# JNP-Solutions/Slacken

Hardware: AMD Instinct MI355X
Metric: classify_throughput_150bp_standard224scale (higher is better)
Workload: dtype u64

## Files before the change

### slacken_amd/csrc/lane.hip

```cpp
#include "engine.h"

#include <algorithm>
#include <cstddef>
#include <cstdio>
#include <cstdlib>

namespace slk {

#ifndef SLK_LANE_LW
#define SLK_LANE_LW 4
#endif
constexpr int LW = SLK_LANE_LW;
constexpr int QCAP = 128;
#ifndef SLK_SBLK
#define SLK_SBLK 5
#endif
constexpr int SBLK = SLK_SBLK;
#ifndef SLK_OMAP
#define SLK_OMAP 12
#endif
constexpr int OMAP = SLK_OMAP;
constexpr int OMAP_CNT_BITS = 10;
constexpr uint32_t OMAP_CNT_MASK = (1u << OMAP_CNT_BITS) - 1;

// ... 96 lines not shown
  for (int s = 0; s < LPB; s++) {
    uint32_t bkt = ((const uint4 *)L->stash)[s * PG + g].x;
    SLK_TUNE(if (dbg & 4) bkt &= 1023u;)
    cell[s] = SLK_PROBE_LOAD((const ulonglong2 *)(cellbase + ((uint64_t)bkt << BUCKET_SHIFT)));
  }
  constexpr uint64_t GROUP_LSB = LPB == 4 ? 0x1111111111111111ULL : 0x0101010101010101ULL;
  int requeued = 0;
#pragma unroll
  for (int s = 0; s < LPB; s++) {
    const uint2 tg = *(const uint2 *)&((const uint4 *)L->stash)[s * PG + g].z;
    const uint64_t want = ((uint64_t)tg.y << 32) | tg.x;
    const bool act = want != NO_TAG;
    const bool e0 = cell[s].x == 0, e1 = cell[s].y == 0;
    const bool m0 = act && !e0 && cell_tag(T.g, cell[s].x) == want;
    const bool m1 = act && !e1 && cell_tag(T.g, cell[s].y) == want;
    if (m0 || m1) L->found[s * PG + g] = (uint32_t)((m0 ? cell[s].x : cell[s].y) & tmask);
    const bool closed = T.g.flag != 0 && c == 0 && (cell[s].x & T.g.flag) == 0;
    const uint64_t B = __ballot(m0 || m1 || e0 || e1 || !act || closed);
    uint64_t any = B;
#pragma unroll
    for (int i = 1; i < LPB; i <<= 1) any |= any >> i;
    if ((any & GROUP_LSB) != GROUP_LSB) {
      const int qj = (qhead + s * PG + g) & (QCAP - 1);
      const uint32_t m_old = L->q_meta[qj];
      const bool again = c == 0 && ((B >> (g * LPB)) & ((1u << LPB) - 1)) == 0 && (int)((m_old >> 20) & 255) < T.max_disp;
      const uint64_t k_old = L->q_key[qj];
      const uint16_t o_old = HITS ? L->q_ord[qj] : (uint16_t)0;
      const uint64_t R = __ballot(again);
      lane_wave_sync();
      if (again) {
        const int slot = (qhead + qn + requeued + __builtin_amdgcn_mbcnt_hi((uint32_t)(R >> 32), __builtin_amdgcn_mbcnt_lo((uint32_t)R, 0))) & (QCAP - 1);
        L->q_key[slot] = k_old;
        L->q_meta[slot] = m_old + (1u << 20);
        if (HITS) L->q_ord[slot] = o_old;
      }
      requeued += __popcll(R);
    }
  }
  lane_wave_sync();
  const int32_t taxon = (int32_t)L->found[lane];
  if (!SLK_TUNE_ON(2)) fold_hit<LONG>(L, ocnt, in, meta, taxon);
  if (HITS && in) {
    const uint64_t at = L->rb[meta & 63] + ord;
    hit_taxon[at] = ext_taxon(T, taxon);
    hit_meta[at] = pack_meta((int32_t)((meta >> 7) & 0x1FFF), 1, (meta >> 6) & 1);
  }
  lane_wave_sync();
  return requeued;
}

#ifndef SLK_STREAM_NT
#define SLK_STREAM_NT 0
#endif
#ifndef SLK_APPLY_ROWS
#define SLK_APPLY_ROWS 4
#endif
template <class T> __device__ __forceinline__ T SLK_STREAM_LOAD(const T *p) {
#if SLK_STREAM_NT
  return __builtin_nontemporal_load(p);
#else
  return *p;
#endif
}
template <class T> __device__ __forceinline__ void SLK_STREAM_STORE(T *p, T v) {
#if SLK_STREAM_NT
  __builtin_nontemporal_store(v, p);
#else
  *p = v;
#endif
}

__device__ __forceinline__ uint64_t lane_readlane64(uint64_t v, int src) {
  uint32_t lo = __builtin_amdgcn_readlane((uint32_t)v, src), hi = __builtin_amdgcn_readlane((uint32_t)(v >> 32), src);
  return ((uint64_t)hi << 32) | lo;
}
__device__ __forceinline__ uint32_t shard_owner(uint64_t key, uint32_t ns) {
  const uint64_t h = fmix64(key);
  return (ns & (ns - 1)) == 0 ? (uint32_t)(h & (ns - 1)) : (uint32_t)(h % ns);
}
__device__ __forceinline__ uint64_t side_load(const ShardIO &S, uint64_t batch, int lane) {
  const uint64_t i = batch * 64 + (uint64_t)lane;
  return i < S.side_n ? (uint64_t)SLK_STREAM_LOAD(&S.side_keys[i]) : 0;
}
__device__ __forceinline__ void side_probe(LaneLds *L, const TableView &T, const ShardIO &S, int lane, uint64_t batch, uint64_t key, int dbg) {
  const uint64_t base = batch * 64;
  if (base >= S.side_n) return;
  const uint64_t i = base + (uint64_t)lane;
  const bool in = i < S.side_n;
  const uint64_t h = fmix64(key);
  uint32_t home;
  uint64_t rem_hi;
  table_slot(T.g, h, home, rem_hi);
  const uint64_t tag = in ? rem_hi : ~0ULL;
  uint4 st;
  st.x = home; st.y = 0; st.z = (uint32_t)tag; st.w = (uint32_t)(tag >> 32);
  ((uint4 *)L->stash)[lane] = st;
  L->found[lane] = 0;
  lane_wave_sync();
  const int g = lane / LPB, c = lane % LPB;
  const uint64_t tmask = (1ULL << T.g.taxon_bits) - 1;
  const char *cellbase = (const char *)T.cells + c * 16;
  ulonglong2 cell[LPB];
#pragma unroll
  for (int s = 0; s < LPB; s++) {
    uint32_t bkt = ((const uint4 *)L->stash)[s * PG + g].x;
    SLK_TUNE(if (dbg & 4) bkt &= 1023u;)
    cell[s] = SLK_PROBE_LOAD((const ulonglong2 *)(cellbase + ((uint64_t)bkt << BUCKET_SHIFT)));
  }
  uint32_t unresolved = 0;
#pragma unroll
  for (int s = 0; s < LPB; s++) {
    const uint2 tg = *(const uint2 *)&((const uint4 *)L->stash)[s * PG + g].z;
    const uint64_t want = ((uint64_t)tg.y << 32) | tg.x;
    const bool act = want != ~0ULL;
    const bool e0 = cell[s].x == 0, e1 = cell[s].y == 0;
    const bool m0 = act && !e0 && cell_tag(T.g, cell[s].x) == want;
    const bool m1 = act && !e1 && cell_tag(T.g, cell[s].y) == want;
    if (m0 || m1) L->found[s * PG + g] = (uint32_t)((m0 ? cell[s].x : cell[s].y) & tmask);
    const bool closed = T.g.flag != 0 && c == 0 && (cell[s].x & T.g.flag) == 0;
    const uint64_t B = __ballot(m0 || m1 || e0 || e1 || !act || closed);
    if (((B >> (g * LPB)) & ((1u << LPB) - 1)) == 0) unresolved |= 1u << s;
  }
  lane_wave_sync();
  int32_t taxon = (int32_t)L->found[lane];
  const uint32_t ur = (uint32_t)__shfl((int)unresolved, (lane % PG) * LPB);
  if (in && ((ur >> (lane / PG)) & 1)) {
    for (int d = 1; d <= T.max_disp; d++) {
      const ulonglong2 *b = (const ulonglong2 *)(T.cells + ((uint64_t)table_bucket(T.g, home, (uint32_t)d) * CELLS));
      const uint64_t want = rem_hi | (uint64_t)d;
      bool has_empty = false, closed = false;
      int32_t hit = 0;
#pragma unroll
      for (int q = 0; q < LPB; q++) {
        const ulonglong2 v = b[q];
        has_empty |= (v.x == 0) | (v.y == 0);
        if (q == 0) closed = T.g.flag != 0 && (v.x & T.g.flag) == 0;
        if (v.x != 0 && cell_tag(T.g, v.x) == want) hit = (int32_t)(v.x & tmask);
        if (v.y != 0 && cell_tag(T.g, v.y) == want) hit = (int32_t)(v.y & tmask);
      }
      if (hit) { taxon = hit; break; }
      if (has_empty || closed) break;
    }
  }
  if (in && !SLK_TUNE_ON(128)) SLK_STREAM_STORE(&S.side_out[i], ext_taxon(T, taxon));
  lane_wave_sync();
}

template <bool HITS>
__device__ __forceinline__ void apply_rows(LaneLds *L, const ApplyJob &J, int lane, uint64_t row0, uint32_t nrows) {
  const uint32_t ns = (uint32_t)J.n_shards;
  constexpr int U = SLK_APPLY_ROWS;
  for (uint32_t b = 0; b < nrows; b += U) {
    uint64_t at[U];
    bool in[U];
#pragma unroll
    for (int u = 0; u < U; u++) {
      in[u] = false;
      at[u] = 0;
      if (b + u < nrows) {
        uint32_t off = 0;
        for (uint32_t sh = 0; sh < ns; sh++) {
          const uint4 e = J.batch_log[(row0 + b + u) * ns + sh];
          const uint32_t cnt = e.z;
          if (cnt == 0) continue;
          if ((uint32_t)lane >= off && (uint32_t)lane < off + cnt) {
            in[u] = true;
            const uint32_t i = (uint32_t)lane - off;
            at[u] = (uint64_t)sh * J.cap + (i < e.w ? e.x + i : e.y + (i - e.w));
          }
          off += cnt;
        }
      }
    }
    uint32_t meta[U];
    int32_t taxon[U];
#pragma unroll
    for (int u = 0; u < U; u++) {
      meta[u] = in[u] ? SLK_STREAM_LOAD(&J.send_meta[at[u]]) : 0u;
      taxon[u] = in[u] ? SLK_STREAM_LOAD(&J.taxa[at[u]]) : 0;
    }
#pragma unroll
    for (int u = 0; u < U; u++) {
      if (b + u < nrows) {
        int32_t t = taxon[u];
        if (in[u]) {
          if (HITS) {
            const uint64_t hat = L->rb[meta[u] & 63] + (meta[u] >> 20);
            J.A.span_taxon[hat] = t;
            J.A.span_meta[hat] = pack_meta((int32_t)((meta[u] >> 7) & 0x1FFF), 1, (meta[u] >> 6) & 1);
          }
          if (J.to_dense != nullptr && t > 0) t = t < J.n_to_dense ? J.to_dense[t] : 0;
        }
        fold_hit<false>(L, nullptr, in[u], meta[u], t);
      }
    }
    lane_wave_sync();
  }
}

template <bool HITS>
__device__ __forceinline__ void emit_batch(LaneLds *L, const FusedArgs &A, const ShardIO &S, const ApplyJob &J, int qhead, int cnt, int lane,
                                           uint64_t row, uint64_t tile, uint32_t &ch_pos, uint32_t &ch_end, uint32_t &side_j, uint64_t &side_key, int dbg) {
  SLK_TUNE(if (dbg & 256) return;)
  const bool in = lane < cnt;
  const int qi = (qhead + lane) & (QCAP - 1);
  const uint64_t key = L->q_key[qi];
  const uint32_t meta = L->q_meta[qi] | (HITS ? (uint32_t)L->q_ord[qi] << 20 : 0u);
  const uint32_t ns = (uint32_t)S.n_shards;
  const uint32_t g = ns == 1 ? 0u : shard_owner(key, ns);
  uint32_t mycount = 0, rank = 0;
  for (uint32_t sh = 0; sh < ns; sh++) {
    const uint64_t m = __ballot(in && g == sh);
    if ((uint32_t)lane == sh) mycount = (uint32_t)__popcll(m);
    if (g == sh) rank = __builtin_amdgcn_mbcnt_hi((uint32_t)(m >> 32), __builtin_amdgcn_mbcnt_lo((uint32_t)m, 0));
  }
  const uint32_t pos = ch_pos, room = ch_end - ch_pos;
  const bool need = (uint32_t)lane < ns && mycount > room;
  unsigned long long got = 0;
  if (need) got = atomicAdd(&S.cursors[lane], (unsigned long long)S.chunk);
  if (side_j < S.side_per_tile) {
    const uint64_t batch = tile * S.side_per_tile + side_j;
    const uint64_t k_now = side_key;
    side_j++;
    if (side_j < S.side_per_tile) side_key = side_load(S, batch + 1, lane);
    side_probe(L, A.T, S, lane, batch, k_now, dbg);
  }
  uint32_t fresh = 0xFFFFFFFFu;
  if (need) {
    if (got + S.chunk <= S.cap) fresh = (uint32_t)got;
    else atomicOr(A.status, 2);
  }
  if ((uint32_t)lane < ns) {
    S.batch_log[row * ns + (uint32_t)lane] = make_uint4(pos, fresh, mycount, room);
    if (need) { ch_pos = fresh == 0xFFFFFFFFu ? 0u : fresh + (mycount - room); ch_end = fresh == 0xFFFFFFFFu ? 0u : fresh + S.chunk; }
    else ch_pos = pos + mycount;
  }
  const uint32_t gpos = (uint32_t)__shfl((int)pos, (int)g), groom = (uint32_t)__shfl((int)room, (int)g), gfresh = (uint32_t)__shfl((int)fresh, (int)g);
  if (in) {
    const bool tail = rank >= groom;
    if ((!tail || gfresh != 0xFFFFFFFFu) && !SLK_TUNE_ON(32)) {
      const uint64_t at = (uint64_t)g * S.cap + (tail ? gfresh + (rank - groom) : gpos + rank);
      SLK_STREAM_STORE(&S.send_keys[at], (int64_t)key);
      SLK_STREAM_STORE(&S.send_meta[at], meta);
    }
  }
  lane_wave_sync();
}

__device__ __forceinline__ uint4 lane_node(const uint4 *nodes, int32_t ntax, int32_t t) {
  return ((uint32_t)t < (uint32_t)ntax) ? nodes[t] : make_uint4(0u, 0x40000000u + (uint32_t)t, 0x40000000u + (uint32_t)t, 0u);
}
__device__ __forceinline__ int lane_code(uint32_t c) {
  const uint32_t VM = (1u << 1) | (1u << 3) | (1u << 7) | (1u << 20) | (1u << 21);
  bool ok = ((c & 0xC0) == 0x40) && ((VM >> (c & 31)) & 1);
  uint32_t t = (c >> 1) & 3;
  t ^= t >> 1;
  return ok ? (int)t : 5;
}

__device__ __forceinline__ uint4 stream_refill(LaneLds *L, int lane, const uint8_t *seq, uint32_t p, uint32_t n, uint32_t room) {
  uint4 v[SBLK];
#pragma unroll
  for (int i = 0; i < SBLK; i++) {
    v[i] = make_uint4(0, 0, 0, 0);
    if (p + 16u * i < n) v[i] = load_block16(seq + p + 16u * i, room - (p + 16u * i));
  }
#pragma unroll
  for (int i = 1; i < SBLK; i++) L->sbuf[(i - 1) * 64 + lane] = v[i];
  return v[0];
}

#ifndef SLK_PACKED_STREAM
#define SLK_PACKED_STREAM 1
#endif
#ifndef SLK_PACK_ROUNDS
#define SLK_PACK_ROUNDS 2
#endif
constexpr uint32_t PACK_MAX_SPAN = 10880;
constexpr uint32_t PACK_WORDS = PACK_MAX_SPAN / 16 + 1;
constexpr int PACK_LOADS = (PACK_MAX_SPAN + 1023) / 1024;
static_assert((size_t)PACK_WORDS * 6 <= (size_t)(SBLK - 1) * 64 * 16, "the packed tile lives in the lane-wise stream's LDS slots");
__device__ __forceinline__ void pack16(const uint4 v, uint32_t &codes, uint32_t &valid) {
  const uint32_t VM = (1u << 1) | (1u << 3) | (1u << 7) | (1u << 20) | (1u << 21);
  const uint32_t w[4] = {v.x, v.y, v.z, v.w};
  codes = 0; valid = 0;
#pragma unroll
  for (int d = 0; d < 4; d++) {
    uint32_t t = (w[d] >> 1) & 0x03030303u;
    t ^= (t >> 1) & 0x01010101u;
    t = (t | (t >> 6) | (t >> 12) | (t >> 18)) & 0xFFu;
    codes |= t << (8 * d);
#pragma unroll
    for (int b = 0; b < 4; b++) {
      const uint32_t c = (w[d] >> (8 * b)) & 0xFFu;
      const uint32_t ok = (((c & 0xC0u) == 0x40u) ? 1u : 0u) & (VM >> (c & 31u));
      valid |= (ok & 1u) << (4 * d + b);
    }
  }
}
__device__ __forceinline__ uint2 packed_take(const uint32_t *pcodes, const uint16_t *pvalid, uint32_t s) {
  const uint32_t wi = s >> 4, bo = s & 15u;
  const uint64_t c64 = (uint64_t)pcodes[wi] | ((uint64_t)pcodes[wi + 1] << 32);
  const uint32_t v32 = (uint32_t)pvalid[wi] | ((uint32_t)pvalid[wi + 1] << 16);
  return make_uint2((uint32_t)(c64 >> (2 * bo)), (v32 >> bo) & 0xFFFFu);
}

#ifndef SLK_LANE_WPS
#define SLK_LANE_WPS 0
#endif
#if SLK_LANE_WPS > 0
#define LANE_BOUNDS __launch_bounds__(LW * 64, SLK_LANE_WPS)
#else
#define LANE_BOUNDS __launch_bounds__(LW * 64) __attribute__((amdgpu_waves_per_eu(4)))
#endif

__device__ __forceinline__ int route_by_length(uint64_t len, uint32_t long_max, uint32_t b0, uint32_t b1, uint32_t b2, uint32_t seg_min_len,
                                               uint32_t wave_min, uint32_t wave_ratio_q10) {
  if (long_max != 0 && len <= long_max) return (len > b0) + (len > b1) + (len > b2);
  if (seg_min_len != 0 && len >= seg_min_len) return HandOn::SEG;
  int c = HandOn::WAVE_CLASSES - 1;
  for (uint64_t b = ((uint64_t)wave_min * wave_ratio_q10) >> 10; c > 0 && len >= b; b = (b * wave_ratio_q10) >> 10) c--;
  return HandOn::WAVE0 + c;
}
__device__ __attribute__((noinline)) void hand_on(unsigned long long *hdr, uint32_t *lists, uint64_t stride, uint64_t long_cap, uint32_t long_max,
                                                  uint32_t b0, uint32_t b1, uint32_t b2, uint32_t seg_min_len, uint32_t wave_min,
                                                  uint32_t wave_ratio_q10, const uint64_t *offsets, const uint64_t *mate_offsets, bool dfr,
                                                  bool too_long, uint64_t r, int lane, bool from_long) {
  const uint64_t DM = __ballot(dfr);
  int route = from_long ? HandOn::LATE : HandOn::REST;
  if (!from_long && dfr && too_long) {
    uint64_t len = offsets[r + 1] - offsets[r];
    if (mate_offsets) len += mate_offsets[r + 1] - mate_offsets[r];
    route = route_by_length(len, long_max, b0, b1, b2, seg_min_len, wave_min, wave_ratio_q10);
  }
  if (!from_long && lane == 0) atomicAdd(&hdr[HandOn::HANDED], (unsigned long long)__popcll(DM));
  for (int l = from_long ? HandOn::LATE : 0; l <= HandOn::LATE; l++) {
    const uint64_t M = __ballot(dfr && route == l);
    if (M == 0) continue;
    const int leader = __ffsll((long long)M) - 1;
    unsigned long long at = 0;
    if (lane == leader) at = atomicAdd(&hdr[HandOn::count_word(l)], (unsigned long long)__popcll(M));
    at = lane_readlane64(at, leader);
    if (dfr && route == l)
      lists[HandOn::list_at(l, stride, long_cap) + at + __builtin_amdgcn_mbcnt_hi((uint32_t)(M >> 32), __builtin_amdgcn_mbcnt_lo((uint32_t)M, 0))] = (uint32_t)r;
  }
}

__global__ void __launch_bounds__(256) route_kernel(FusedArgs A) {
// ... 223 lines not shown
      if (paired) n2 = (uint32_t)(A.mate_offsets[r + 1] - A.mate_offsets[r]);
    }
    bool too_long = have && ((uint64_t)n + n2 > max_len);
    bool fin = !have || too_long;
    uint64_t row = 0, row0 = 0;
    if (MODE == LANE_EMIT && tile < etiles) row = row0 = (span_region(A.offsets, A.mate_offsets, tile * 64) >> 6) + tile;
    const uint64_t rbase = (HITS && have) ? span_region(A.offsets, A.mate_offsets, r) : 0;
    if (HITS && MODE != LANE_EMIT) L->rb[lane] = rbase;
#pragma unroll
    for (int s = 0; s < OMAP; s++) L->omap[s * 64 + lane] = 0;
    if (LONG) {
#pragma unroll
      for (int s = 0; s < OMAP; s++) ocnt[s * 64 + lane] = 0;
    }
    L->o_flags[lane] = 0;
    if (MODE == LANE_EMIT && tile < atiles) {
      const uint64_t r2 = tile * 64 + lane;
      const bool have2 = r2 < Jp->A.R;
      const uint2 tr = Jp->tile_rows[tile];
      if (HITS) L->rb[lane] = have2 ? span_region(Jp->A.offsets, Jp->A.mate_offsets, r2) : 0;
      lane_wave_sync();
      apply_rows<HITS>(L, *Jp, lane, tr.x, tr.y);
      const bool dfr2 = have2 && (Jp->defer[r2] != 0 || (L->o_flags[lane] & 0x80000000u));
      const uint64_t DM = __ballot(dfr2);
      if (DM != 0 && lane == 0) atomicAdd(Jp->n_deferred, (unsigned long long)__popcll(DM));
      if (have2) {
        if (dfr2) {
          Jp->defer[r2] = 1;
          if (Jp->A.out_nh) Jp->A.out_nh[r2] = 0;
          if (HITS) Jp->A.span_count[r2] = 0;
        } else {
          const int2 ri = Jp->read_info[r2];
          resolve_lane<HITS, false>(L, nullptr, Jp->A, lane, r2, L->o_flags[lane], ri.x, ri.y, 0, dbg);
        }
      }
      lane_wave_sync();
    }
    uint32_t pos = 0;
    int mate = 0;
    uint32_t cur = 0, b1 = 0, b2 = 0, b3 = 0;
    int sb = 1;
    bool packed = false;
    uint32_t s0 = 0;
    uint32_t *const pcodes = (uint32_t *)L->sbuf;
    uint16_t *const pvalid = (uint16_t *)(pcodes + PACK_WORDS);
    constexpr bool CAN_PACK = SLK_PACKED_STREAM && !LONG && MODE == LANE_LOCAL;
    if (CAN_PACK && !paired) {
      const uint64_t t0 = tile * 64, t1 = min(A.R, t0 + 64);
      const uint64_t span_o = A.offsets[t0], span = A.offsets[t1] - span_o;
      if (span <= PACK_MAX_SPAN && __ballot(!fin) != 0) {
        packed = true;
        s0 = have ? (uint32_t)(A.offsets[r] - span_o) : 0;
        const uint8_t *tb = A.bases + span_o;
        const uint32_t troom = clamp_room(bases_end - span_o), sp = (uint32_t)span;
        constexpr int PG0 = (PACK_LOADS + SLK_PACK_ROUNDS - 1) / SLK_PACK_ROUNDS;
#pragma unroll
        for (int j0 = 0; j0 < PACK_LOADS; j0 += PG0) {
          uint4 v[PG0];
#pragma unroll
          for (int j = 0; j < PG0; j++) {
            const uint32_t cb = (uint32_t)(j0 + j) * 1024u + (uint32_t)lane * 16u;
            v[j] = make_uint4(0, 0, 0, 0);
            if (j0 + j < PACK_LOADS && cb < sp) v[j] = load_block16(tb + cb, troom - cb);
          }
#pragma unroll
          for (int j = 0; j < PG0; j++) {
            const uint32_t cb = (uint32_t)(j0 + j) * 1024u + (uint32_t)lane * 16u;
            if (j0 + j < PACK_LOADS && cb < sp + 16u) {
              uint32_t cw, vw;
              pack16(v[j], cw, vw);
              pcodes[cb >> 4] = cw;
              pvalid[cb >> 4] = (uint16_t)vw;
            }
          }
        }
        lane_wave_sync();
      }
    }
    if (!fin && n > 0) {
      if (CAN_PACK && packed) {
        const uint2 pk = packed_take(pcodes, pvalid, s0);
        cur = pk.x; b1 = pk.y;
      } else {
        uint4 v = stream_refill(L, lane, seq, 0, n, room);
        cur = v.x; b1 = v.y; b2 = v.z; b3 = v.w;
      }
    }
    int run_class = 0;
    uint32_t run_len = 0, nvalid = 0;
    uint64_t fwd = 0, rc = 0;
    uint64_t k1 = ~0ULL, p1 = ~0ULL, p2 = ~0ULL, m41 = ~0ULL;
    uint64_t pre = ~0ULL;
    uint64_t cur_val = 0;
    int32_t cur_run = 0;
    bool first = true, have_last = false;
    uint64_t last_key = 0;
    int32_t total = 0, np = 0, nhits = 0;
    uint32_t side_j = (MODE == LANE_EMIT && S.side_n != 0 && tile < etiles) ? 0u : 0xFFFFFFFFu;
    uint64_t side_key = (MODE == LANE_EMIT && S.side_n != 0 && S.side_per_tile != 0 && tile < etiles) ? side_load(S, tile * S.side_per_tile, lane) : 0;
    int qn = 0;
    int qhead = 0;
    int tphase = 0;

    const uint32_t VM = (1u << 1) | (1u << 3) | (1u << 7) | (1u << 20) | (1u << 21);
    while (__ballot(!fin) != 0) {
      if (!W5 && tphase == 0) pre = ~0ULL;
      const bool act = !fin;
      const bool is_end = pos >= n;
      bool okc;
      uint32_t t;
      if (CAN_PACK && packed) {
        t = cur & 3u;
        okc = (b1 & 1u) != 0;
      } else {
        const uint32_t c = cur & 0xFF;
        okc = ((c & 0xC0) == 0x40) && ((VM >> (c & 31)) & 1);
        t = (c >> 1) & 3;
        t ^= t >> 1;
      }
      const int cls = is_end ? -1 : (okc ? 1 : 0);
      const bool run_end = act && run_len > 0 && cls != run_class;
      const bool seqrun = run_class == 1 && nvalid >= (uint32_t)k;
      const bool seq_close = run_end && seqrun;
      const bool amb_close = run_end && !seqrun && run_len >= (uint32_t)k;
      const int32_t ord0 = nhits;
      total += amb_close ? (int32_t)run_len - (k - 1) : 0;
      if (HITS && amb_close) {
        A.span_meta[rbase + ord0] = pack_meta((int32_t)run_len - (k - 1), 2, 0);
        A.span_taxon[rbase + ord0] = -1;
      }
      nhits += amb_close ? 1 : 0;
      first = first && !amb_close;
      const uint64_t ekey = cur_val;
      const int32_t ekmers = cur_run;
      run_len = run_end ? 0u : run_len;
      const bool proc = act && !is_end;
      const bool new_run = proc && run_len == 0;
      run_class = new_run ? cls : run_class;
      nvalid = new_run ? 0u : nvalid;
      cur_run = (new_run || seq_close) ? 0 : cur_run;
      run_len += proc ? 1u : 0u;
      const bool nt = proc && okc;
      nvalid += nt ? 1u : 0u;
      fwd = (fwd << 2) | ((uint64_t)t << P.sh);
      rc = ((rc >> 2) | ((uint64_t)(3 - t) << 62)) & P.keep;
      const bool havekey = nt && nvalid >= (uint32_t)m;
      const uint64_t canon = (P.canonical && rc < fwd) ? rc : fwd;
      const uint64_t key = (canon ^ P.xmask) & P.smask;
      uint64_t minv;
      if (W5) {
        const uint64_t p = lmin64(key, k1);
        const uint64_t m4 = lmin64(p, p2);
        minv = lmin64(key, m41);
        k1 = key; p2 = p1; p1 = p; m41 = m4;
      } else {
        const uint64_t kk = havekey ? key : ~0ULL;
        pre = lmin64(pre, kk);
        minv = (tphase == w - 1) ? pre : lmin64(pre, win[(tphase + 1) * 64 + lane]);
        win[tphase * 64 + lane] = kk;
      }
      const bool havewin = havekey && nvalid >= (uint32_t)k;
      const bool start = havewin && cur_run == 0;
      const bool same = havewin && cur_run != 0 && minv == cur_val;
      const bool change = havewin && cur_run != 0 && minv != cur_val;
      const bool emit = seq_close || change;
      cur_val = (start || change) ? minv : cur_val;
      cur_run = (start || change) ? 1 : (same ? cur_run + 1 : cur_run);
      pos += proc ? 1u : 0u;
      const bool refill = proc && (pos & 15) == 0;
      if (CAN_PACK && packed) {
        cur = proc ? (cur >> 2) : cur;
        b1 = proc ? (b1 >> 1) : b1;
        if (__ballot(refill) != 0) {
          if (refill && pos < n) {
            const uint2 pk = packed_take(pcodes, pvalid, s0 + pos);
            cur = pk.x; b1 = pk.y;
          }
        }
      } else {
        const bool nextdw = proc && (pos & 3) == 0;
        cur = nextdw ? b1 : (proc ? (cur >> 8) : cur);
        b1 = nextdw ? b2 : b1;
        b2 = nextdw ? b3 : b2;
        if (__ballot(refill) != 0) {
          if (refill) {
            if (pos < n) {
              uint4 v;
              if (sb < SBLK) { v = L->sbuf[(sb - 1) * 64 + lane]; sb++; }
              else { v = stream_refill(L, lane, seq, pos, n, room); sb = 1; }
              cur = v.x; b1 = v.y; b2 = v.z; b3 = v.w;
            }
          }
        }
      }
      const bool at_end = act && is_end;
      if (__ballot(at_end) != 0) {
        if (at_end) {
          if (mate == 0 && paired) {
            if (HITS) {
              const int32_t ordb = ord0 + ((amb_close || emit) ? 1 : 0);
              A.span_meta[rbase + ordb] = pack_meta(-(k - 1), 3, 0);
              A.span_taxon[rbase + ordb] = -2;
            }
            nhits++;
            first = false;
            mate = 1;
            const uint64_t o2 = A.mate_offsets[r];
            seq = A.mate_bases + o2; n = (uint32_t)(A.mate_offsets[r + 1] - o2); room = clamp_room(mates_end - o2); pos = 0;
            if (n > 0) {
              uint4 v = stream_refill(L, lane, seq, 0, n, room);
              sb = 1;
              cur = v.x; b1 = v.y; b2 = v.z; b3 = v.w;
            }
          } else {
            fin = true;
          }
        }
      }
      if (!W5) {
        if (tphase == w - 1) {
          uint64_t sm = ~0ULL;
          for (int j = w - 1; j >= 0; j--) { sm = lmin64(sm, win[j * 64 + lane]); win[j * 64 + lane] = sm; }
          tphase = 0;
        } else {
          tphase++;
        }
      }
      const bool distinct = emit && (first || !(have_last && ekey == last_key));
      last_key = emit ? ekey : last_key;
      have_last = have_last || emit;
      first = first && !emit;
      total += emit ? ekmers : 0;
      np += emit ? 1 : 0;
      nhits += emit ? 1 : 0;
      uint64_t E = __ballot(emit);
      if (E != 0) {
        if (emit) {
          int slot = (qhead + qn + __builtin_amdgcn_mbcnt_hi((uint32_t)(E >> 32), __builtin_amdgcn_mbcnt_lo((uint32_t)E, 0))) & (QCAP - 1);
          L->q_key[slot] = ekey;
          if (HITS) L->q_ord[slot] = (uint16_t)ord0;
          L->q_meta[slot] = (uint32_t)lane | (distinct ? 64u : 0u) | ((uint32_t)ekmers << 7);
        }
        qn += __popcll(E);
        while (qn >= 64) {
          lane_wave_sync();
          int back = 0;
          if (MODE == LANE_EMIT) emit_batch<HITS>(L, A, S, *Jp, qhead, 64, lane, row++, tile, ch_pos, ch_end, side_j, side_key, dbg);
          else if (!SLK_TUNE_ON(1)) back = probe_batch<HITS, LONG>(L, ocnt, A.T, qhead, qn, 64, lane, dbg, A.span_meta, A.span_taxon);
          qhead = (qhead + 64) & (QCAP - 1);
          qn += back - 64;
        }
      }
    }
    while (qn > 0) {
      lane_wave_sync();
      const int cnt = min(qn, 64);
      int back = 0;
      if (MODE == LANE_EMIT) emit_batch<HITS>(L, A, S, *Jp, qhead, cnt, lane, row++, tile, ch_pos, ch_end, side_j, side_key, dbg);
      else if (!SLK_TUNE_ON(1)) back = probe_batch<HITS, LONG>(L, ocnt, A.T, qhead, qn, cnt, lane, dbg, A.span_meta, A.span_taxon);
      qhead = (qhead + cnt) & (QCAP - 1);
      qn += back - cnt;
    }
    lane_wave_sync();
    if (MODE == LANE_EMIT) {
      if (tile < etiles) {
        if (have) S.read_info[r] = make_int2(total, nhits);
        if (lane == 0) S.tile_rows[tile] = make_uint2((uint32_t)row0, (uint32_t)(row - row0));
      }
      while (side_j < S.side_per_tile) {
        const uint64_t batch = tile * S.side_per_tile + side_j;
        const uint64_t k_now = side_key;
        side_j++;
        if (side_j < S.side_per_tile) side_key = side_load(S, batch + 1, lane);
        side_probe(L, A.T, S, lane, batch, k_now, dbg);
      }
    }

    if (MODE == LANE_LOCAL) {
      const uint32_t oflags = have ? L->o_flags[lane] : 0u;
      const bool dfr = have && (too_long || (oflags & 0x80000000u));
      if (__ballot(dfr) != 0)
        hand_on(A.hand_hdr, A.hand_lists, A.hand_stride, A.hand_long_cap, A.long_max, A.long_bound[0], A.long_bound[1], A.long_bound[2],
                A.seg_min_len, A.wave_min, A.wave_ratio_q10, A.offsets, A.mate_offsets, dfr, too_long, r, lane, LONG);
      if (have && !dfr) resolve_lane<HITS, LONG>(L, ocnt, A, lane, r, oflags, total, nhits, np, dbg);
    } else {
      if (have && too_long) defer[r] = 1;
    }
    lane_wave_sync();
  }
  if (MODE == LANE_EMIT) {
    for (uint32_t sh = 0; sh < (uint32_t)S.n_shards; sh++) {
      const uint32_t p0 = __builtin_amdgcn_readlane(ch_pos, sh), p1 = __builtin_amdgcn_readlane(ch_end, sh);
      for (uint32_t i = p0 + (uint32_t)lane; i < p1; i += 64) S.send_keys[(uint64_t)sh * S.cap + i] = 0;
    }
  }
}

template <bool W5, int MODE, bool HITS, bool LONG>
__global__ void LANE_BOUNDS lane_kernel(FusedArgs A, ShardIO S, int32_t *defer, uint32_t max_len, int dbg) {
  lane_body<W5, MODE, HITS, LONG>(A, S, nullptr, defer, max_len, dbg);
}
template <bool W5, bool HITS>
__global__ void LANE_BOUNDS lane_step_kernel(FusedArgs A, ShardIO S, ApplyJob J, int32_t *defer, uint32_t max_len, int dbg) {
  lane_body<W5, LANE_EMIT, HITS, false>(A, S, &J, defer, max_len, dbg);
}

static size_t lane_lds_per_wave(bool hits, bool w5, int w, bool lng) {
  return (hits ? sizeof(LaneLds) : offsetof(LaneLds, rb)) + (w5 ? 0 : (size_t)w * 64 * sizeof(uint64_t)) + (lng ? (size_t)OMAP * 64 * sizeof(uint32_t) : 0);
}

template <bool HITS, bool LONG>
static void launch_lane_mode(const FusedArgs &A, int32_t *defer, uint32_t max_len, hipStream_t s) {
  if (A.R == 0) return;
  const bool w5 = A.P.w == 5;
  const size_t per_wave = lane_lds_per_wave(HITS, w5, A.P.w, LONG);
  static const int extra_lds = getenv("SLK_LANE_EXTRA_LDS") ? atoi(getenv("SLK_LANE_EXTRA_LDS")) : 0;
  size_t lds = per_wave * LW + (size_t)extra_lds;
  uint64_t tiles = (A.R + 63) / 64;
  uint64_t blocks = (tiles + LW - 1) / LW;
  static const int bpc = getenv("SLK_LANE_BLOCKS_PER_CU") ? atoi(getenv("SLK_LANE_BLOCKS_PER_CU")) : 0;
  if (bpc > 0 && blocks > (uint64_t)256 * bpc) blocks = (uint64_t)256 * bpc;
  if (LONG && blocks > 256 * 5) blocks = 256 * 5;
  dim3 g((unsigned)blocks), b(LW * 64);
#ifdef SLK_TUNING
  static const int dbg = getenv("SLK_DEBUG_ABLATE") ? atoi(getenv("SLK_DEBUG_ABLATE")) : 0;
#else
  const int dbg = 0;
#endif
  static bool occ_printed = false;
  if (getenv("SLK_DEBUG_OCC") && !occ_printed) {
    occ_printed = true;
    int nb = 0;
    (void)hipOccupancyMaxActiveBlocksPerMultiprocessor(&nb, w5 ? (const void *)lane_kernel<true, LANE_LOCAL, HITS, LONG> : (const void *)lane_kernel<false, LANE_LOCAL, HITS, LONG>, LW * 64, lds);
    fprintf(stderr, "[slk] lane kernel: %zu B LDS per block, %d blocks (%d waves) resident per CU\n", lds, nb, nb * LW);
  }
  if (w5) hipLaunchKernelGGL((lane_kernel<true, LANE_LOCAL, HITS, LONG>), g, b, lds, s, A, ShardIO{}, defer, max_len, dbg);
  else hipLaunchKernelGGL((lane_kernel<false, LANE_LOCAL, HITS, LONG>), g, b, lds, s, A, ShardIO{}, defer, max_len, dbg);
}

void launch_lane(const FusedArgs &A, int32_t *defer, uint32_t max_len, hipStream_t s) {
  if (A.span_taxon) launch_lane_mode<true, false>(A, defer, max_len, s);
  else launch_lane_mode<false, false>(A, defer, max_len, s);
}
void launch_lane_long(const FusedArgs &A, uint32_t max_len, hipStream_t s) {
  if (A.span_taxon) launch_lane_mode<true, true>(A, nullptr, max_len, s);
  else launch_lane_mode<false, true>(A, nullptr, max_len, s);
}

template <bool W5, bool HITS>
static void launch_step_mode(const FusedArgs &A, const ShardIO &S, const ApplyJob &J, int32_t *defer, uint32_t max_len, hipStream_t s) {
  const uint64_t tiles = std::max((A.R + 63) / 64, (J.A.R + 63) / 64);
  if (tiles == 0) return;
  const size_t lds = lane_lds_per_wave(HITS, W5, A.P.w, false) * LW;
  static int resident[2][2] = {{0, 0}, {0, 0}};
  static int cus = 0;
  if (cus == 0) {
    int dev = 0;
    (void)hipGetDevice(&dev);
    if (hipDeviceGetAttribute(&cus, hipDeviceAttributeMultiprocessorCount, dev) != hipSuccess || cus <= 0) cus = 256;
  }
  int nb = W5 ? resident[1][HITS] : 0;
  if (nb == 0) {
    if (hipOccupancyMaxActiveBlocksPerMultiprocessor(&nb, (const void *)lane_step_kernel<W5, HITS>, LW * 64, lds) != hipSuccess || nb <= 0) nb = 4;
    if (W5) resident[1][HITS] = nb;
  }
  static const int bpc = getenv("SLK_STEP_BLOCKS_PER_CU") ? atoi(getenv("SLK_STEP_BLOCKS_PER_CU")) : 0;
  if (bpc > 0) nb = bpc;
  const uint64_t blocks = std::min<uint64_t>((tiles + LW - 1) / LW, (uint64_t)cus * nb);
#ifdef SLK_TUNING
  static const int dbg = getenv("SLK_DEBUG_ABLATE") ? atoi(getenv("SLK_DEBUG_ABLATE")) : 0;
#else
  const int dbg = 0;
#endif
  hipLaunchKernelGGL((lane_step_kernel<W5, HITS>), dim3((unsigned)blocks), dim3(LW * 64), lds, s, A, S, J, defer, max_len, dbg);
}
void launch_lane_step(const FusedArgs &A, const ShardIO &S, const ApplyJob &J, int32_t *defer, uint32_t max_len, hipStream_t s) {
  const bool hits = A.R ? A.span_taxon != nullptr : J.A.span_taxon != nullptr;
  if (A.P.w == 5) { if (hits) launch_step_mode<true, true>(A, S, J, defer, max_len, s); else launch_step_mode<true, false>(A, S, J, defer, max_len, s); }
  else { if (hits) launch_step_mode<false, true>(A, S, J, defer, max_len, s); else launch_step_mode<false, false>(A, S, J, defer, max_len, s); }
}

}
```

Baseline: 1142.

## Carry unresolved side-key lookups to later cooperative rounds instead of per-lane displacement loops

Side-key probes that miss in their home bucket no longer walk the displacement chain serially per lane. They are queued in an LDS ring placed over the taxon map and re-probed cooperatively at the next displacement, 64 at a time, in later batches or in a drain loop at tile end. This removes divergent, uncoalesced serial loads from the probe path. The cost is extra LDS traffic and bookkeeping, plus reuse of the omap region, which must not be live during the emit phase.

```diff
diff --git a/slacken_amd/csrc/lane.hip b/slacken_amd/csrc/lane.hip
--- a/slacken_amd/csrc/lane.hip
+++ b/slacken_amd/csrc/lane.hip
@@ -202,18 +202,25 @@
   const uint64_t i = batch * 64 + (uint64_t)lane;
   return i < S.side_n ? (uint64_t)SLK_STREAM_LOAD(&S.side_keys[i]) : 0;
 }
-__device__ __forceinline__ void side_probe(LaneLds *L, const TableView &T, const ShardIO &S, int lane, uint64_t batch, uint64_t key, int dbg) {
-  const uint64_t base = batch * 64;
-  if (base >= S.side_n) return;
-  const uint64_t i = base + (uint64_t)lane;
-  const bool in = i < S.side_n;
+constexpr int CARRY_CAP = 128;
+__device__ __forceinline__ uint64_t *carry_key(LaneLds *L) { return (uint64_t *)L->omap; }
+__device__ __forceinline__ uint32_t *carry_batch(LaneLds *L) { return L->omap + 2 * CARRY_CAP; }
+__device__ __forceinline__ uint16_t *carry_ld(LaneLds *L) { return (uint16_t *)(L->omap + 3 * CARRY_CAP); }
+static_assert(CARRY_CAP * (8 + 4 + 2) <= OMAP * 64 * 4 && offsetof(LaneLds, omap) % 8 == 0, "the ring of carried lookups lies over the taxon map");
+#ifdef SLK_TUNING
+__device__ unsigned long long slk_tune_side[2];
+#endif
+
+__device__ __forceinline__ void side_coop(LaneLds *L, const TableView &T, const ShardIO &S, int lane, bool in, uint64_t key, uint32_t j, uint32_t ld,
+                                          uint64_t tile_first, int c_head, int &c_n, int dbg) {
+  const uint32_t disp = ld >> 6;
   const uint64_t h = fmix64(key);
   uint32_t home;
   uint64_t rem_hi;
   table_slot(T.g, h, home, rem_hi);
-  const uint64_t tag = in ? rem_hi : ~0ULL;
+  const uint64_t tag = in ? rem_hi + disp : ~0ULL;
   uint4 st;
-  st.x = home; st.y = 0; st.z = (uint32_t)tag; st.w = (uint32_t)(tag >> 32);
+  st.x = table_bucket(T.g, home, disp); st.y = 0; st.z = (uint32_t)tag; st.w = (uint32_t)(tag >> 32);
   ((uint4 *)L->stash)[lane] = st;
   L->found[lane] = 0;
   lane_wave_sync();
@@ -242,28 +249,53 @@
     if (((B >> (g * LPB)) & ((1u << LPB) - 1)) == 0) unresolved |= 1u << s;
   }
   lane_wave_sync();
-  int32_t taxon = (int32_t)L->found[lane];
+  const int32_t taxon = (int32_t)L->found[lane];
   const uint32_t ur = (uint32_t)__shfl((int)unresolved, (lane % PG) * LPB);
-  if (in && ((ur >> (lane / PG)) & 1)) {
-    for (int d = 1; d <= T.max_disp; d++) {
-      const ulonglong2 *b = (const ulonglong2 *)(T.cells + ((uint64_t)table_bucket(T.g, home, (uint32_t)d) * CELLS));
-      const uint64_t want = rem_hi | (uint64_t)d;
-      bool has_empty = false, closed = false;
-      int32_t hit = 0;
-#pragma unroll
-      for (int q = 0; q < LPB; q++) {
-        const ulonglong2 v = b[q];
-        has_empty |= (v.x == 0) | (v.y == 0);
-        if (q == 0) closed = T.g.flag != 0 && (v.x & T.g.flag) == 0;
-        if (v.x != 0 && cell_tag(T.g, v.x) == want) hit = (int32_t)(v.x & tmask);
-        if (v.y != 0 && cell_tag(T.g, v.y) == want) hit = (int32_t)(v.y & tmask);
-      }
-      if (hit) { taxon = hit; break; }
-      if (has_empty || closed) break;
-    }
-  }
-  if (in && !SLK_TUNE_ON(128)) SLK_STREAM_STORE(&S.side_out[i], ext_taxon(T, taxon));
+  const bool open = in && ((ur >> (lane / PG)) & 1);
+  const bool again = open && disp < (uint32_t)T.max_disp && !SLK_TUNE_ON(512);
+  SLK_TUNE(if (dbg & 1024) {
+    const uint64_t O = __ballot(open);
+    if (lane == 0 && __builtin_amdgcn_readfirstlane(disp) == 0) { atomicAdd(&slk_tune_side[0], 1ULL); if (O != 0) atomicAdd(&slk_tune_side[1], 1ULL); }
+  })
+  if (in && !again && !SLK_TUNE_ON(128))
+    SLK_STREAM_STORE(&S.side_out[(tile_first + j) * 64 + (ld & 63u)], ext_taxon(T, taxon));
+  const uint64_t R = __ballot(again);
+  if (R != 0) {
+    if (again) {
+      const int slot = (c_head + c_n + __builtin_amdgcn_mbcnt_hi((uint32_t)(R >> 32), __builtin_amdgcn_mbcnt_lo((uint32_t)R, 0))) & (CARRY_CAP - 1);
+      carry_key(L)[slot] = key;
+      carry_batch(L)[slot] = j;
+      carry_ld(L)[slot] = (uint16_t)(ld + 64u);
+    }
+    c_n += __popcll(R);
+  }
   lane_wave_sync();
+}
+
+__device__ __forceinline__ void side_probe(LaneLds *L, const TableView &T, const ShardIO &S, int lane, uint64_t tile_first, uint32_t j, uint64_t key,
+                                           bool fresh, int &c_head, int &c_n, int dbg) {
+  for (;;) {
+    const int cnt = c_n >= 64 ? 64 : (fresh ? 0 : c_n);
+    bool in;
+    uint64_t k = key;
+    uint32_t jj = j, ld = (uint32_t)lane;
+    if (cnt != 0) {
+      const int ci = (c_head + lane) & (CARRY_CAP - 1);
+      in = lane < cnt;
+      k = in ? carry_key(L)[ci] : 0;
+      jj = carry_batch(L)[ci];
+      ld = in ? (uint32_t)carry_ld(L)[ci] : (uint32_t)lane;
+      c_head = (c_head + cnt) & (CARRY_CAP - 1);
+      c_n -= cnt;
+    } else {
+      if (!fresh) return;
+      const uint64_t base = (tile_first + j) * 64;
+      if (base >= S.side_n) return;
+      in = base + (uint64_t)lane < S.side_n;
+    }
+    side_coop(L, T, S, lane, in, k, jj, ld, tile_first, c_head, c_n, dbg);
+    if (cnt == 0) return;
+  }
 }
 
 template <bool HITS>
@@ -320,7 +352,7 @@
 
 template <bool HITS>
 __device__ __forceinline__ void emit_batch(LaneLds *L, const FusedArgs &A, const ShardIO &S, const ApplyJob &J, int qhead, int cnt, int lane,
-                                           uint64_t row, uint64_t tile, uint32_t &ch_pos, uint32_t &ch_end, uint32_t &side_j, uint64_t &side_key, int dbg) {
+                                           uint64_t row, uint64_t tile, uint32_t &ch_pos, uint32_t &ch_end, uint32_t &side_j, uint64_t &side_key, int &c_head, int &c_n, int dbg) {
   SLK_TUNE(if (dbg & 256) return;)
   const bool in = lane < cnt;
   const int qi = (qhead + lane) & (QCAP - 1);
@@ -339,11 +371,12 @@
   unsigned long long got = 0;
   if (need) got = atomicAdd(&S.cursors[lane], (unsigned long long)S.chunk);
   if (side_j < S.side_per_tile) {
-    const uint64_t batch = tile * S.side_per_tile + side_j;
+    const uint64_t tile_first = tile * S.side_per_tile;
+    const uint32_t j = side_j;
     const uint64_t k_now = side_key;
     side_j++;
-    if (side_j < S.side_per_tile) side_key = side_load(S, batch + 1, lane);
-    side_probe(L, A.T, S, lane, batch, k_now, dbg);
+    if (side_j < S.side_per_tile) side_key = side_load(S, tile_first + side_j, lane);
+    side_probe(L, A.T, S, lane, tile_first, j, k_now, true, c_head, c_n, dbg);
   }
   uint32_t fresh = 0xFFFFFFFFu;
   if (need) {
@@ -789,6 +822,7 @@
     int32_t total = 0, np = 0, nhits = 0;
     uint32_t side_j = (MODE == LANE_EMIT && S.side_n != 0 && tile < etiles) ? 0u : 0xFFFFFFFFu;
     uint64_t side_key = (MODE == LANE_EMIT && S.side_n != 0 && S.side_per_tile != 0 && tile < etiles) ? side_load(S, tile * S.side_per_tile, lane) : 0;
+    int c_head = 0, c_n = 0;
     int qn = 0;
     int qhead = 0;
     int tphase = 0;
@@ -936,7 +970,7 @@
         while (qn >= 64) {
           lane_wave_sync();
           int back = 0;
-          if (MODE == LANE_EMIT) emit_batch<HITS>(L, A, S, *Jp, qhead, 64, lane, row++, tile, ch_pos, ch_end, side_j, side_key, dbg);
+          if (MODE == LANE_EMIT) emit_batch<HITS>(L, A, S, *Jp, qhead, 64, lane, row++, tile, ch_pos, ch_end, side_j, side_key, c_head, c_n, dbg);
           else if (!SLK_TUNE_ON(1)) back = probe_batch<HITS, LONG>(L, ocnt, A.T, qhead, qn, 64, lane, dbg, A.span_meta, A.span_taxon);
           qhead = (qhead + 64) & (QCAP - 1);
           qn += back - 64;
@@ -947,7 +981,7 @@
       lane_wave_sync();
       const int cnt = min(qn, 64);
       int back = 0;
-      if (MODE == LANE_EMIT) emit_batch<HITS>(L, A, S, *Jp, qhead, cnt, lane, row++, tile, ch_pos, ch_end, side_j, side_key, dbg);
+      if (MODE == LANE_EMIT) emit_batch<HITS>(L, A, S, *Jp, qhead, cnt, lane, row++, tile, ch_pos, ch_end, side_j, side_key, c_head, c_n, dbg);
       else if (!SLK_TUNE_ON(1)) back = probe_batch<HITS, LONG>(L, ocnt, A.T, qhead, qn, cnt, lane, dbg, A.span_meta, A.span_taxon);
       qhead = (qhead + cnt) & (QCAP - 1);
       qn += back - cnt;
@@ -958,12 +992,17 @@
         if (have) S.read_info[r] = make_int2(total, nhits);
         if (lane == 0) S.tile_rows[tile] = make_uint2((uint32_t)row0, (uint32_t)(row - row0));
       }
-      while (side_j < S.side_per_tile) {
-        const uint64_t batch = tile * S.side_per_tile + side_j;
+      for (;;) {
+        const bool fresh = side_j < S.side_per_tile;
+        const uint64_t tile_first = tile * S.side_per_tile;
+        const uint32_t j = side_j;
         const uint64_t k_now = side_key;
-        side_j++;
-        if (side_j < S.side_per_tile) side_key = side_load(S, batch + 1, lane);
-        side_probe(L, A.T, S, lane, batch, k_now, dbg);
+        if (fresh) {
+          side_j++;
+          if (side_j < S.side_per_tile) side_key = side_load(S, tile_first + side_j, lane);
+        }
+        side_probe(L, A.T, S, lane, tile_first, j, k_now, fresh, c_head, c_n, dbg);
+        if (!fresh) break;
       }
     }
 
@@ -1072,3 +1111,9 @@
 }
 
 }
+
+#ifdef SLK_TUNING
+extern "C" int slk_tune_side_counts(unsigned long long *out) {
+  return (int)hipMemcpyFromSymbol(out, HIP_SYMBOL(slk::slk_tune_side), 2 * sizeof(unsigned long long));
+}
+#endif
```

Measured after the change: 1142, median of 2. No clear change (-0.0%).

## Stage batch log in LDS, reorder side-probe store, single-wait stream refill

Applied to the files above, without the earlier changes.

apply_rows now copies a block of the batch log into LDS with a few coalesced loads per lane. It then locates each lane's entry from LDS and batches the send_meta/taxa gathers and to_dense lookups, instead of rereading global log entries per row and per shard. emit_batch delays the side-probe result store until after the cursor atomic resolves, so the atomic's latency can overlap the probe. stream_refill gains a fast path for the emit mode: when the whole block lies within bounds it uses plain 16-byte memcpy loads in place of the guarded load_block16. The staging reuses the LDS region that holds the queue, stash and stream slots, which relies on those being dead during apply.

```diff
diff --git a/slacken_amd/csrc/lane.hip b/slacken_amd/csrc/lane.hip
--- a/slacken_amd/csrc/lane.hip
+++ b/slacken_amd/csrc/lane.hip
@@ -202,9 +202,9 @@
   const uint64_t i = batch * 64 + (uint64_t)lane;
   return i < S.side_n ? (uint64_t)SLK_STREAM_LOAD(&S.side_keys[i]) : 0;
 }
-__device__ __forceinline__ void side_probe(LaneLds *L, const TableView &T, const ShardIO &S, int lane, uint64_t batch, uint64_t key, int dbg) {
+__device__ __forceinline__ bool side_probe(LaneLds *L, const TableView &T, const ShardIO &S, int lane, uint64_t batch, uint64_t key, int dbg, int32_t &answer) {
   const uint64_t base = batch * 64;
-  if (base >= S.side_n) return;
+  if (base >= S.side_n) return false;
   const uint64_t i = base + (uint64_t)lane;
   const bool in = i < S.side_n;
   const uint64_t h = fmix64(key);
@@ -262,10 +262,107 @@
       if (has_empty || closed) break;
     }
   }
-  if (in && !SLK_TUNE_ON(128)) SLK_STREAM_STORE(&S.side_out[i], ext_taxon(T, taxon));
+  answer = ext_taxon(T, taxon);
   lane_wave_sync();
-}
-
+  return in && !SLK_TUNE_ON(128);
+}
+__device__ __forceinline__ void side_store(const ShardIO &S, int lane, uint64_t batch, bool mine, int32_t answer) {
+  if (mine) SLK_STREAM_STORE(&S.side_out[batch * 64 + (uint64_t)lane], answer);
+}
+
+#ifndef SLK_APPLY_STAGE
+#define SLK_APPLY_STAGE 1
+#endif
+#ifndef SLK_APPLY_STAGE_LOADS
+#define SLK_APPLY_STAGE_LOADS 4
+#endif
+constexpr int APPLY_STAGE_LOADS = SLK_APPLY_STAGE_LOADS;
+constexpr uint32_t APPLY_STAGE = APPLY_STAGE_LOADS * 64;
+static_assert(APPLY_STAGE * sizeof(uint4) <= offsetof(LaneLds, omap), "a stage of the log lies over the queue, the stash and the read stream's slots");
+#if SLK_APPLY_STAGE
+template <bool HITS>
+__device__ __forceinline__ void apply_rows(LaneLds *L, const ApplyJob &J, int lane, uint64_t row0, uint32_t nrows) {
+  const uint32_t ns = (uint32_t)J.n_shards;
+  constexpr int U = SLK_APPLY_ROWS;
+  uint4 *const stg = (uint4 *)L;
+  uint32_t srows = APPLY_STAGE / ns;
+  if (srows > (uint32_t)U) srows -= srows % U;
+  for (uint32_t s0 = 0; s0 < nrows; s0 += srows) {
+    const uint32_t sr = min(srows, nrows - s0), ne = sr * ns;
+    const uint4 *const src = J.batch_log + (row0 + s0) * ns;
+    {
+      uint4 v[APPLY_STAGE_LOADS];
+#pragma unroll
+      for (int j = 0; j < APPLY_STAGE_LOADS; j++) {
+        const uint32_t i = (uint32_t)j * 64u + (uint32_t)lane;
+        v[j] = make_uint4(0, 0, 0, 0);
+        if (i < ne) v[j] = src[i];
+      }
+#pragma unroll
+      for (int j = 0; j < APPLY_STAGE_LOADS; j++) stg[j * 64 + lane] = v[j];
+    }
+    lane_wave_sync();
+    auto locate = [&](uint32_t b, uint64_t *at, bool *in) {
+      uint32_t off[U];
+#pragma unroll
+      for (int u = 0; u < U; u++) { in[u] = false; at[u] = 0; off[u] = 0; }
+      for (uint32_t sh = 0; sh < ns; sh++) {
+#pragma unroll
+        for (int u = 0; u < U; u++) {
+          const uint4 e = stg[min(b + u, sr - 1) * ns + sh];
+          const uint32_t cnt = b + u < sr ? e.z : 0u;
+          const uint32_t i = (uint32_t)lane - off[u];
+          if (i < cnt) {
+            in[u] = true;
+            at[u] = (uint64_t)sh * J.cap + (i < e.w ? e.x + i : e.y + (i - e.w));
+          }
+          off[u] += cnt;
+        }
+      }
+    };
+    auto fetch = [&](const uint64_t *at, const bool *in, uint32_t *meta, int32_t *taxon) {
+#pragma unroll
+      for (int u = 0; u < U; u++) {
+        meta[u] = in[u] ? SLK_STREAM_LOAD(&J.send_meta[at[u]]) : 0u;
+        taxon[u] = in[u] ? SLK_STREAM_LOAD(&J.taxa[at[u]]) : 0;
+      }
+    };
+    auto fold = [&](uint32_t b, const bool *in, const uint32_t *meta, const int32_t *taxon) {
+      int32_t t[U];
+#pragma unroll
+      for (int u = 0; u < U; u++) t[u] = in[u] ? taxon[u] : 0;
+      if (J.to_dense != nullptr) {
+        int32_t d[U];
+#pragma unroll
+        for (int u = 0; u < U; u++) d[u] = J.to_dense[(t[u] > 0 && t[u] < J.n_to_dense) ? t[u] : 0];
+#pragma unroll
+        for (int u = 0; u < U; u++) t[u] = t[u] > 0 ? (t[u] < J.n_to_dense ? d[u] : 0) : t[u];
+      }
+#pragma unroll
+      for (int u = 0; u < U; u++) {
+        if (b + u < sr) {
+          if (HITS && in[u]) {
+            const uint64_t hat = L->rb[meta[u] & 63] + (meta[u] >> 20);
+            J.A.span_taxon[hat] = taxon[u];
+            J.A.span_meta[hat] = pack_meta((int32_t)((meta[u] >> 7) & 0x1FFF), 1, (meta[u] >> 6) & 1);
+          }
+          fold_hit<false>(L, nullptr, in[u], meta[u], t[u]);
+        }
+      }
+    };
+    for (uint32_t b = 0; b < sr; b += U) {
+      uint64_t at[U];
+      bool in[U];
+      uint32_t meta[U];
+      int32_t taxon[U];
+      locate(b, at, in);
+      fetch(at, in, meta, taxon);
+      fold(b, in, meta, taxon);
+    }
+    lane_wave_sync();
+  }
+}
+#else
 template <bool HITS>
 __device__ __forceinline__ void apply_rows(LaneLds *L, const ApplyJob &J, int lane, uint64_t row0, uint32_t nrows) {
   const uint32_t ns = (uint32_t)J.n_shards;
@@ -317,7 +414,11 @@
     lane_wave_sync();
   }
 }
-
+#endif
+
+#ifndef SLK_EMIT_CURSOR_FIRST
+#define SLK_EMIT_CURSOR_FIRST 1
+#endif
 template <bool HITS>
 __device__ __forceinline__ void emit_batch(LaneLds *L, const FusedArgs &A, const ShardIO &S, const ApplyJob &J, int qhead, int cnt, int lane,
                                            uint64_t row, uint64_t tile, uint32_t &ch_pos, uint32_t &ch_end, uint32_t &side_j, uint64_t &side_key, int dbg) {
@@ -338,18 +439,29 @@
   const bool need = (uint32_t)lane < ns && mycount > room;
   unsigned long long got = 0;
   if (need) got = atomicAdd(&S.cursors[lane], (unsigned long long)S.chunk);
+  uint64_t side_batch = 0;
+  int32_t side_answer = 0;
+  bool side_mine = false;
   if (side_j < S.side_per_tile) {
-    const uint64_t batch = tile * S.side_per_tile + side_j;
+    side_batch = tile * S.side_per_tile + side_j;
     const uint64_t k_now = side_key;
     side_j++;
-    if (side_j < S.side_per_tile) side_key = side_load(S, batch + 1, lane);
-    side_probe(L, A.T, S, lane, batch, k_now, dbg);
+    if (side_j < S.side_per_tile) side_key = side_load(S, side_batch + 1, lane);
+    side_mine = side_probe(L, A.T, S, lane, side_batch, k_now, dbg, side_answer);
+#if !SLK_EMIT_CURSOR_FIRST
+    side_store(S, lane, side_batch, side_mine, side_answer);
+#else
+    asm volatile("" : "+v"(side_answer));
+#endif
   }
   uint32_t fresh = 0xFFFFFFFFu;
   if (need) {
     if (got + S.chunk <= S.cap) fresh = (uint32_t)got;
     else atomicOr(A.status, 2);
   }
+#if SLK_EMIT_CURSOR_FIRST
+  side_store(S, lane, side_batch, side_mine, side_answer);
+#endif
   if ((uint32_t)lane < ns) {
     S.batch_log[row * ns + (uint32_t)lane] = make_uint4(pos, fresh, mycount, room);
     if (need) { ch_pos = fresh == 0xFFFFFFFFu ? 0u : fresh + (mycount - room); ch_end = fresh == 0xFFFFFFFFu ? 0u : fresh + S.chunk; }
@@ -378,12 +490,24 @@
   return ok ? (int)t : 5;
 }
 
+#ifndef SLK_REFILL_ONE_WAIT
+#define SLK_REFILL_ONE_WAIT 1
+#endif
+template <bool ONE_WAIT>
 __device__ __forceinline__ uint4 stream_refill(LaneLds *L, int lane, const uint8_t *seq, uint32_t p, uint32_t n, uint32_t room) {
   uint4 v[SBLK];
-#pragma unroll
-  for (int i = 0; i < SBLK; i++) {
-    v[i] = make_uint4(0, 0, 0, 0);
-    if (p + 16u * i < n) v[i] = load_block16(seq + p + 16u * i, room - (p + 16u * i));
+  if (ONE_WAIT && room >= p + 16u * SBLK) {
+#pragma unroll
+    for (int i = 0; i < SBLK; i++) {
+      v[i] = make_uint4(0, 0, 0, 0);
+      if (p + 16u * i < n) __builtin_memcpy(&v[i], seq + p + 16u * i, 16);
+    }
+  } else {
+#pragma unroll
+    for (int i = 0; i < SBLK; i++) {
+      v[i] = make_uint4(0, 0, 0, 0);
+      if (p + 16u * i < n) v[i] = load_block16(seq + p + 16u * i, room - (p + 16u * i));
+    }
   }
 #pragma unroll
   for (int i = 1; i < SBLK; i++) L->sbuf[(i - 1) * 64 + lane] = v[i];
@@ -773,7 +897,7 @@
         const uint2 pk = packed_take(pcodes, pvalid, s0);
         cur = pk.x; b1 = pk.y;
       } else {
-        uint4 v = stream_refill(L, lane, seq, 0, n, room);
+        uint4 v = stream_refill<SLK_REFILL_ONE_WAIT && MODE == LANE_EMIT>(L, lane, seq, 0, n, room);
         cur = v.x; b1 = v.y; b2 = v.z; b3 = v.w;
       }
     }
@@ -878,7 +1002,7 @@
             if (pos < n) {
               uint4 v;
               if (sb < SBLK) { v = L->sbuf[(sb - 1) * 64 + lane]; sb++; }
-              else { v = stream_refill(L, lane, seq, pos, n, room); sb = 1; }
+              else { v = stream_refill<SLK_REFILL_ONE_WAIT && MODE == LANE_EMIT>(L, lane, seq, pos, n, room); sb = 1; }
               cur = v.x; b1 = v.y; b2 = v.z; b3 = v.w;
             }
           }
@@ -899,7 +1023,7 @@
             const uint64_t o2 = A.mate_offsets[r];
             seq = A.mate_bases + o2; n = (uint32_t)(A.mate_offsets[r + 1] - o2); room = clamp_room(mates_end - o2); pos = 0;
             if (n > 0) {
-              uint4 v = stream_refill(L, lane, seq, 0, n, room);
+              uint4 v = stream_refill<SLK_REFILL_ONE_WAIT && MODE == LANE_EMIT>(L, lane, seq, 0, n, room);
               sb = 1;
               cur = v.x; b1 = v.y; b2 = v.z; b3 = v.w;
             }
@@ -963,7 +1087,9 @@
         const uint64_t k_now = side_key;
         side_j++;
         if (side_j < S.side_per_tile) side_key = side_load(S, batch + 1, lane);
-        side_probe(L, A.T, S, lane, batch, k_now, dbg);
+        int32_t answer = 0;
+        const bool mine = side_probe(L, A.T, S, lane, batch, k_now, dbg, answer);
+        side_store(S, lane, batch, mine, answer);
       }
     }
 
```

Measured after the change: 1131 before, 1131 after. About the same (-0.0%).
